# haoheliu/voicefixer

Hardware: AMD Instinct MI355X
Metric: seconds-of-44.1kHz-audio restored per wall-second (higher is better)
Workload: dtype f32

## Files before the change

### voicefixer_amd/csrc/vfx_common.h

```cpp
#pragma once
#include <hip/hip_runtime.h>
#include <stdint.h>
#include <atomic>
#include "../../include/vfx_hip.h"

extern __attribute__((visibility("hidden"))) std::atomic<uint64_t> g_vfx_launches;

#define VFX_LAUNCHED() (g_vfx_launches.fetch_add(1, std::memory_order_relaxed))

static inline int vfx_last_error() {
    hipError_t e = hipGetLastError();
    return e == hipSuccess ? VFX_OK : (int)e;
}

__attribute__((visibility("hidden"))) int vfx_zero_u32(void* p, size_t bytes, hipStream_t s);

#ifdef VFX_DEV
#include <stdlib.h>
#define VFX_DEV_ENV(name) getenv(name)
#else
#define VFX_DEV_ENV(name) (static_cast<const char*>(nullptr))
#endif

static inline bool vfx_aligned16(const void* p) { return (reinterpret_cast<uintptr_t>(p) & 15u) == 0; }

__device__ __forceinline__ float vfx_lrelu(float v, float slope) { return v > 0.f ? v : v * slope; }

__device__ __forceinline__ float vfx_post(float v, int act, float slope) {
    switch (act) {
        case VFX_POST_LRELU: return vfx_lrelu(v, slope);
        case VFX_POST_ELU: return v > 0.f ? v : expm1f(v);
        case VFX_POST_TANH: return tanhf(v);
        case VFX_POST_SIGMOID: return 1.f / (1.f + expf(-v));
        case VFX_POST_LRELU_SNAKE: { float u = vfx_lrelu(v, slope); return u + sinf(u); }
        default: return v;
    }
}
```

### voicefixer_amd/csrc/vfx_convwg.inc

```

static void convwg_fold_blocks(ConvArgs& a, dim3& grid, int gy) {
    static const bool off = VFX_DEV_ENV("VFX_WINO_MFOLD") && atoi(VFX_DEV_ENV("VFX_WINO_MFOLD")) == 0;
    a.nph_fold = 0;
    if (gy > 1 && a.xcd_chunk > 0 && !off) {
        a.nph_fold = gy;
        grid = dim3(grid.x * gy, 1, grid.z);
    }
}

#ifndef VFX_WG4_OCC
#define VFX_WG4_OCC 2
#endif
#ifndef VFX_WG4_ABL
#define VFX_WG4_ABL 0
#endif
#ifndef VFX_WG4_SPEC2_OCC
#define VFX_WG4_SPEC2_OCC 2
#endif
template <int WGM, int WGP, bool D1 = false, int XD = 2, bool PRE = true, int SPEC = 0>
__global__ __launch_bounds__(256, (SPEC == 2 && WGM == 4) ? VFX_WG4_SPEC2_OCC : VFX_WG4_OCC) void convwg4_kernel(const ConvArgs a) {
    static_assert(WGM * WGP == 4, "four waves");
    static_assert(SPEC == 0 || (SPEC == 1 && PRE) || (SPEC == 2 && D1 && !PRE), "specialised instances");
    constexpr bool ZSTART = SPEC != 0;
    static_assert(XD == 2 || XD == 3, "prefetch distance");
    constexpr int XSETS = XD - 1;
    constexpr int KC = 16, NSTEP = KC / 2;
    constexpr int BM = 32 * WGM, BQ = 32 * WGP;
    constexpr int CG = 256 / BQ;
    constexpr int NSLOT = KC / CG;
    constexpr int SPAN = NSTEP / NSLOT;
    constexpr int PLANE = KC * BQ;
    constexpr int BUF = 6 * PLANE;
    static_assert(CG % 2 == 0 && (SPAN == 2 || SPAN == 4), "staging map");
    extern __shared__ __attribute__((aligned(16))) float smem[];

    const int tid = threadIdx.x, lane = tid & 63;
    const int wave = __builtin_amdgcn_readfirstlane(tid >> 6);
    const int lo = lane & 31, hi = lane >> 5;
    const int wm = wave / WGP, wp = wave % WGP;
    int bx = blockIdx.x;
    int mblk = blockIdx.y;
    if (a.xcd_chunk > 0) {
        int k = bx >> 3;
        if (a.nph_fold > 1) {
            const int t = k / a.nph_fold;
            mblk = k - t * a.nph_fold;
            k = t;
        }
        bx = (bx & 7) * a.xcd_chunk + k;
        if (bx >= a.ntiles_l) return;
    }
    const int m0 = mblk * BM;
    const int b = blockIdx.z;
    const int d = D1 ? 1 : a.wg_d;
    const float inv_d = 1.0f / (float)d;
    const int Lrow = a.x_rows ? __builtin_amdgcn_readfirstlane(a.x_rows[b]) : a.Lin;
    const int Q0 = bx * BQ;
    {
        const int nblk = fast_div(Lrow + 4 * d - 1, 4 * d, 0.25f * inv_d);
        if (Q0 >= nblk * d) return;
    }
    if (a.stagger) {
        const int lin = blockIdx.x + gridDim.x * (blockIdx.y + gridDim.y * blockIdx.z);
        if (lin < a.stagger_wgs) {
            const int slot = __builtin_amdgcn_s_getreg((3 << 11) | 4) & 15;
            for (int i = 0; i < slot * a.stagger; ++i) __builtin_amdgcn_s_sleep(127);
        }
    }
    DBG_T(dbg_t0);
#if VFX_ABL & 8
    unsigned long long dbg_bar = 0;
#define WG4_SYNC() do { DBG_T(b0_); __syncthreads(); DBG_T(b1_); dbg_bar += b1_ - b0_; } while (0)
#else
#define WG4_SYNC() do { if (!(VFX_WG4_ABL & 16)) __syncthreads(); } while (0)
#endif
    const int xcs = (int)a.x_cs;
    auto quad_q = [&](int Q) {
        if constexpr (D1) return 4 * Q;
        const int blk = fast_div(Q, d, inv_d);
        return 4 * d * blk + (Q - blk * d);
    };
    const bool has_tail = D1 && (Lrow & 3) != 0 && (Lrow >> 2) >= Q0 && (Lrow >> 2) < Q0 + BQ;

    const int sq = tid % BQ, cg = tid / BQ;
    int xvoff[6];
    bool xin[4] = {true, true, true, true};
    {
        const int q = quad_q(Q0 + sq);
#pragma unroll
        for (int j = 0; j < 6; ++j) {
            const int p = q + (j - 1) * d;
            xvoff[j] = (p >= 0 && p < Lrow) ? (cg * xcs + p) * 4 : VFX_W_OOB;
        }
        if constexpr (D1) {
#pragma unroll
            for (int i = 0; i < 4; ++i) xin[i] = q + i < Lrow;
        }
    }
    const __amdgpu_buffer_rsrc_t xrsrc = __builtin_amdgcn_make_buffer_rsrc(
        const_cast<float*>(a.x) + (long long)b * a.x_bs, (short)0, 0x7fffffff, 0x00020000);
    const float slope = a.pre_act == VFX_PRE_LRELU ? a.pre_slope : 1.f;
    auto x_soff = [&](int v) { return v * KC * xcs * 4; };
    const int wcol = BQ == 32 ? sq : ((sq & ~63) | ((sq + 32 * (cg & 1)) & 63));
    float* const wbase = smem + cg * BQ + wcol;

    float xv[XSETS][NSLOT][6];
    auto x_load_part = [&](auto set_tag, int j, int part, int s0) {
        constexpr int SET = decltype(set_tag)::value;
        const int so = s0 + j * CG * xcs * 4;
        if constexpr (D1) {
            if (part == 0) {
                const u32x4 r = __builtin_amdgcn_raw_buffer_load_b128(xrsrc, xvoff[1], so, 0);
                xv[SET][j][1] = __uint_as_float(r.x); xv[SET][j][2] = __uint_as_float(r.y);
                xv[SET][j][3] = __uint_as_float(r.z); xv[SET][j][4] = __uint_as_float(r.w);
            } else if (part == 1) {
                xv[SET][j][0] = __uint_as_float(__builtin_amdgcn_raw_buffer_load_b32(xrsrc, xvoff[0], so, 0));
            } else if (part == 2) {
                xv[SET][j][5] = __uint_as_float(__builtin_amdgcn_raw_buffer_load_b32(xrsrc, xvoff[5], so, 0));
            }
        } else {
            xv[SET][j][part] = __uint_as_float(__builtin_amdgcn_raw_buffer_load_b32(xrsrc, xvoff[part], so, 0));
        }
    };
    auto x_load = [&](auto set_tag, int v) {
        const int s0 = x_soff(v);
#pragma unroll
        for (int j = 0; j < NSLOT; ++j)
#pragma unroll
            for (int t = 0; t < 6; ++t) x_load_part(set_tag, j, t, s0);
    };
    auto x_transform = [&](auto set_tag, int j, float (&V)[6]) {
        constexpr int SET = decltype(set_tag)::value;
        float e[6];
#pragma unroll
        for (int t = 0; t < 6; ++t) {
            e[t] = PRE ? fmaxf(xv[SET][j][t], xv[SET][j][t] * slope) : xv[SET][j][t];
            if constexpr (D1) {
                if (t >= 1 && t <= 4) e[t] = xin[t - 1] ? e[t] : 0.f;
            }
        }
        const float s1 = fmaf(-4.f, e[2], e[4]), s2 = fmaf(-4.f, e[1], e[3]);
        const float s3 = e[4] - e[2], s4 = e[3] - e[1];
        V[0] = fmaf(4.f, e[0], fmaf(-5.f, e[2], e[4]));
        V[1] = s1 + s2;
        V[2] = s1 - s2;
        V[3] = fmaf(2.f, s4, s3);
        V[4] = fmaf(-2.f, s4, s3);
        V[5] = fmaf(4.f, e[1], fmaf(-5.f, e[3], e[5]));
    };
    auto x_write = [&](auto set_tag, float* dst) {
#pragma unroll
        for (int j = 0; j < NSLOT; ++j) {
            float V[6];
            x_transform(set_tag, j, V);
#pragma unroll
            for (int k = 0; k < 6; ++k) dst[j * CG * BQ + k * PLANE] = V[k];
        }
    };

    const __amdgpu_buffer_rsrc_t wrsrc =
        __builtin_amdgcn_make_buffer_rsrc(const_cast<float*>(a.wd), (short)0, 0x7fffffff, 0x00020000);
    const int avoff = ((m0 + wm * 32 + lo) * 8 + 4 * hi) * 4;
    const int gstride = a.Cout * 32;
    const int pstride = (a.CinPad >> 3) * gstride;
    float4 aw[2][6];
    auto a_goff = [&](int vg) { return (VFX_WG4_ABL & 1) ? 0 : vg * gstride; };
    auto a_load_one = [&](auto set_tag, int k, int goff) {
        constexpr int SET = decltype(set_tag)::value;
        const u32x4 r = __builtin_amdgcn_raw_buffer_load_b128(wrsrc, avoff, k * pstride + goff, 0);
        aw[SET][k] = make_float4(__uint_as_float(r.x), __uint_as_float(r.y), __uint_as_float(r.z), __uint_as_float(r.w));
    };

    const int row0 = m0 + wm * 32;
    int rv[4];
    int rvq = VFX_W_OOB;
    {
        const int q = quad_q(Q0 + wp * 32 + lo);
#pragma unroll
        for (int i = 0; i < 4; ++i) rv[i] = q + i * d < Lrow ? (4 * hi * (int)a.r_cs + q + i * d) * 4 : VFX_W_OOB;
        if constexpr (D1) {
            const bool full = q + 3 < Lrow;
            rvq = (full && a.res) ? rv[0] : VFX_W_OOB;
#pragma unroll
            for (int i = 0; i < 4; ++i) rv[i] = full ? VFX_W_OOB : rv[i];
        }
    }
    f32x16 acc[6];
    u32x4 rq[(D1 && SPEC == 0) ? 16 : 1];
    const __amdgpu_buffer_rsrc_t rrsrc = __builtin_amdgcn_make_buffer_rsrc(
        const_cast<float*>(a.res ? a.res : a.x) + (long long)b * a.r_bs, (short)0, 0x7fffffff, 0x00020000);
    const __amdgpu_buffer_rsrc_t brsrc = __builtin_amdgcn_make_buffer_rsrc(
        const_cast<float*>(a.bias ? a.bias : a.x), (short)0, 0x7fffffff, 0x00020000);
    u32x4 bq[4];
    {
        const int bvoff = a.bias ? (row0 + 4 * hi) * 4 : VFX_W_OOB;
#pragma unroll
        for (int g = 0; g < 4; ++g) bq[g] = __builtin_amdgcn_raw_buffer_load_b128(brsrc, bvoff, g * 32, 0);
    }
    using X0 = std::integral_constant<int, 0>;
    using X1 = std::integral_constant<int, XSETS - 1>;
#if VFX_ABL & 8
    __builtin_amdgcn_sched_barrier(0);
#endif
    DBG_T(dbg_tr);
#if VFX_ABL & 8
    __builtin_amdgcn_sched_barrier(0);
#endif
    x_load(X0{}, 0);
#pragma unroll
    for (int k = 0; k < 6; ++k) a_load_one(std::integral_constant<int, 0>{}, k, a_goff(0));
#if VFX_ABL & 8
    __builtin_amdgcn_sched_barrier(0);
#endif
    DBG_T(dbg_ts);
#if VFX_ABL & 8
    __builtin_amdgcn_sched_barrier(0);
#endif
    if constexpr (SPEC == 0) {
        const int cs4 = (int)a.r_cs * 4;
        if constexpr (D1) {
#pragma unroll
            for (int r = 0; r < 16; ++r)
                rq[r] = __builtin_amdgcn_raw_buffer_load_b128(rrsrc, rvq, (row0 + (r & 3) + 8 * (r >> 2)) * cs4, 0);
        } else if (a.res) {
#pragma unroll
            for (int r = 0; r < 16; ++r) {
                const int soff = (row0 + (r & 3) + 8 * (r >> 2)) * cs4;
                acc[0][r] = __uint_as_float(__builtin_amdgcn_raw_buffer_load_b32(rrsrc, rv[0], soff, 0));
                acc[1][r] = __uint_as_float(__builtin_amdgcn_raw_buffer_load_b32(rrsrc, rv[1], soff, 0));
                acc[3][r] = __uint_as_float(__builtin_amdgcn_raw_buffer_load_b32(rrsrc, rv[2], soff, 0));
                acc[5][r] = __uint_as_float(__builtin_amdgcn_raw_buffer_load_b32(rrsrc, rv[3], soff, 0));
            }
        } else {
#pragma unroll
            for (int r = 0; r < 16; ++r) { acc[0][r] = 0.f; acc[1][r] = 0.f; acc[3][r] = 0.f; acc[5][r] = 0.f; }
        }
    }
    __builtin_amdgcn_sched_barrier(0);
    DBG_T(dbg_ta);
    auto acc_start = [&]() {
        if constexpr (ZSTART) return;
        if constexpr (D1 && SPEC == 0) {
#pragma unroll
            for (int r = 0; r < 16; ++r) {
                acc[0][r] = __uint_as_float(rq[r].x); acc[1][r] = __uint_as_float(rq[r].y);
                acc[3][r] = __uint_as_float(rq[r].z); acc[5][r] = __uint_as_float(rq[r].w);
            }
        }
        if (D1 && has_tail && a.res) {
            const int cs4 = (int)a.r_cs * 4;
#pragma unroll 1
            for (int r = 0; r < 16; ++r) {
                const int soff = (row0 + (r & 3) + 8 * (r >> 2)) * cs4;
                const float t0 = __uint_as_float(__builtin_amdgcn_raw_buffer_load_b32(rrsrc, rv[0], soff, 0));
                const float t1 = __uint_as_float(__builtin_amdgcn_raw_buffer_load_b32(rrsrc, rv[1], soff, 0));
                const float t2 = __uint_as_float(__builtin_amdgcn_raw_buffer_load_b32(rrsrc, rv[2], soff, 0));
                const float t3 = __uint_as_float(__builtin_amdgcn_raw_buffer_load_b32(rrsrc, rv[3], soff, 0));
                acc[0][r] += t0; acc[1][r] += t1; acc[3][r] += t2; acc[5][r] += t3;
            }
        }
        if (!a.res) {
#pragma unroll
            for (int g = 0; g < 4; ++g)
#pragma unroll
                for (int e = 0; e < 4; ++e) {
                    const int r = 4 * g + e;
                    acc[0][r] = 0.f;
                    acc[1][r] = __uint_as_float(e == 0 ? bq[g].x : (e == 1 ? bq[g].y : (e == 2 ? bq[g].z : bq[g].w)));
                    acc[2][r] = 0.f; acc[3][r] = 0.f; acc[4][r] = 0.f; acc[5][r] = 0.f;
                }
            return;
        }
#pragma unroll
        for (int g = 0; g < 4; ++g) {
#pragma unroll
            for (int e = 0; e < 4; ++e) {
                const int r = 4 * g + e;
                const float bb = __uint_as_float(e == 0 ? bq[g].x : (e == 1 ? bq[g].y : (e == 2 ? bq[g].z : bq[g].w)));
                const float t0 = acc[0][r] + bb, t1 = acc[1][r] + bb, t2 = acc[3][r] + bb, t3 = acc[5][r] + bb;
                const float m3 = 0.5f * (t2 - t1);
                const float m1 = 2.f * t1 - t2;
                acc[0][r] = t0 - m1 - m3;
                acc[1][r] = m1;
                acc[2][r] = 0.f;
                acc[3][r] = m3;
                acc[4][r] = 0.f;
                acc[5][r] = t3 - m1 - 8.f * m3;
            }
        }
    };

    const int bcol = BQ == 32 ? lo : ((wp * 32 + lo + 32 * hi) & 63);
    const int boffs = hi * BQ + bcol;

    f32x16 biasv;
    if constexpr (ZSTART) {
#pragma unroll
        for (int g = 0; g < 4; ++g) {
            biasv[4 * g + 0] = __uint_as_float(bq[g].x); biasv[4 * g + 1] = __uint_as_float(bq[g].y);
            biasv[4 * g + 2] = __uint_as_float(bq[g].z); biasv[4 * g + 3] = __uint_as_float(bq[g].w);
        }
    }
    auto mma_chunk = [&](auto set_tag, auto first_tag, const float* xs, float* wdst, int xchunk, int agrp0, int glast) {
        constexpr bool FIRST = decltype(first_tag)::value;
        const float* bp = xs + boffs;
        const int agrp1 = a_goff(min(agrp0 + 1, glast)), agrp2 = a_goff(min(agrp0 + 2, glast));
        float bf[6];
#pragma unroll
        for (int k = 0; k < 6; ++k) bf[k] = bp[k * PLANE];
        const int xs0 = x_soff(xchunk);
        float V[6];
#pragma unroll
        for (int u = 0; u < NSTEP; ++u) {
            const int el = u / SPAN, ph = u % SPAN;
#pragma unroll
            for (int k = 0; k < 6; ++k) {
                constexpr bool ST = !(VFX_WG4_ABL & 8), LD = !(VFX_WG4_ABL & 2);
                if constexpr (SPAN == 4) {
                    if (ST && ph == 0 && k == 0) x_transform(set_tag, el, V);
                    if (ST && ph == 0 && k < 3) wdst[el * CG * BQ + k * PLANE] = V[k];
                    if (ST && ph == 1 && k < 3) wdst[el * CG * BQ + (k + 3) * PLANE] = V[k + 3];
                    if (LD && ph == 2 && k < 3) x_load_part(set_tag, el, k, xs0);
                    if (LD && ph == 3 && k < 3) x_load_part(set_tag, el, k + 3, xs0);
                } else {
                    if (ST && ph == 0 && k == 0) x_transform(set_tag, el, V);
                    if (ST && ph == 0) wdst[el * CG * BQ + k * PLANE] = V[k];
                    if (LD && ph == 1) x_load_part(set_tag, el, k, xs0);
                }
                if (u == 0) a_load_one(std::integral_constant<int, 1>{}, k, agrp1);
                if (u == 4) a_load_one(std::integral_constant<int, 0>{}, k, agrp2);
                const float4 av4 = (u < 4) ? aw[0][k] : aw[1][k];
                const int kk = u & 3;
                const float av = kk == 0 ? av4.x : (kk == 1 ? av4.y : (kk == 2 ? av4.z : av4.w));
                if constexpr (FIRST) {
                    if (u == 0) {
                        const f32x16 zero16 = {0.f, 0.f, 0.f, 0.f, 0.f, 0.f, 0.f, 0.f, 0.f, 0.f, 0.f, 0.f, 0.f, 0.f, 0.f, 0.f};
                        acc[k] = __builtin_amdgcn_mfma_f32_32x32x2f32(av, bf[k], k == 1 ? biasv : zero16, 0, 0, 0);
                    } else {
                        acc[k] = __builtin_amdgcn_mfma_f32_32x32x2f32(av, bf[k], acc[k], 0, 0, 0);
                    }
                } else {
                    acc[k] = __builtin_amdgcn_mfma_f32_32x32x2f32(av, bf[k], acc[k], 0, 0, 0);
                }
                if (u < NSTEP - 1 && !(VFX_WG4_ABL & 4)) bf[k] = bp[k * PLANE + (u + 1) * 2 * BQ];
                __builtin_amdgcn_sched_barrier(0);
            }
        }
    };

    const int S = a.Cin / KC;
    const int glast = 2 * S - 1;
    x_write(X0{}, wbase);
    DBG_T(dbg_tb);
    x_load(X0{}, S > 1 ? 1 : 0);
    if constexpr (XSETS == 2) x_load(X1{}, min(2, S - 1));
    __builtin_amdgcn_sched_barrier(0);
    acc_start();
    DBG_T(dbg_tc);
    WG4_SYNC();
    DBG_T(dbg_t1);
    using NotFirst = std::false_type;
    int s_begin = 0;
    if constexpr (ZSTART) {
        mma_chunk(X0{}, std::true_type{}, smem, wbase + BUF, min(XD, S - 1), 0, glast);
        WG4_SYNC();
        mma_chunk(X1{}, NotFirst{}, smem + BUF, wbase, min(1 + XD, S - 1), 2, glast);
        WG4_SYNC();
        s_begin = 2;
    }
#pragma unroll 1
    for (int s = s_begin; s < S; s += 2) {
        mma_chunk(X0{}, NotFirst{}, smem, wbase + BUF, min(s + XD, S - 1), 2 * s, glast);
        WG4_SYNC();
        mma_chunk(X1{}, NotFirst{}, smem + BUF, wbase, min(s + 1 + XD, S - 1), 2 * s + 2, glast);
        WG4_SYNC();
    }
    DBG_T(dbg_t2);

    const __amdgpu_buffer_rsrc_t yrsrc = __builtin_amdgcn_make_buffer_rsrc(
        a.y + (long long)b * a.y_bs, (short)0, 0x7fffffff, 0x00020000);
    const int ycs4 = (int)a.y_cs * 4;
    const int post = a.post_act;
    const float ps = a.post_slope;
    int yv[4];
    int yvq = VFX_W_OOB;
    {
        const int q = quad_q(Q0 + wp * 32 + lo);
#pragma unroll
        for (int i = 0; i < 4; ++i) yv[i] = q + i * d < Lrow ? (4 * hi * (int)a.y_cs + q + i * d) * 4 : VFX_W_OOB;
        if constexpr (D1) {
            const bool full = q + 3 < Lrow;
            yvq = full ? yv[0] : VFX_W_OOB;
#pragma unroll
            for (int i = 0; i < 4; ++i) yv[i] = full ? VFX_W_OOB : yv[i];
        }
    }
    auto store4 = [&](const float (&v)[4], int soff) {
        if constexpr (D1) {
            u32x4 u;
            u.x = __float_as_uint(v[0]); u.y = __float_as_uint(v[1]); u.z = __float_as_uint(v[2]); u.w = __float_as_uint(v[3]);
            __builtin_amdgcn_raw_buffer_store_b128(u, yrsrc, yvq, soff, 0);
        }
        if (!D1 || has_tail) {
#pragma unroll
            for (int i = 0; i < 4; ++i) __builtin_amdgcn_raw_buffer_store_b32(__float_as_uint(v[i]), yrsrc, yv[i], soff, 0);
        }
    };
    auto outs = [&](int r, float (&y)[4]) {
        const float p12 = acc[1][r] + acc[2][r], m12 = acc[1][r] - acc[2][r];
        const float p34 = acc[3][r] + acc[4][r], m34 = acc[3][r] - acc[4][r];
        y[0] = (acc[0][r] + p12) + p34;
        y[1] = fmaf(2.f, m34, m12);
        y[2] = fmaf(4.f, p34, p12);
        y[3] = fmaf(8.f, m34, m12) + acc[5][r];
    };
    if constexpr (SPEC == 1) {
#pragma unroll
        for (int r = 0; r < 16; ++r) {
            const int soff = (row0 + (r & 3) + 8 * (r >> 2)) * ycs4;
            float y[4];
            outs(r, y);
#pragma unroll
            for (int i = 0; i < 4; ++i) y[i] = fmaxf(y[i], y[i] * ps);
            store4(y, soff);
        }
    } else if constexpr (SPEC == 2) {
        const int cs4 = (int)a.r_cs * 4;
        const int qe = quad_q(Q0 + wp * 32 + lo);
        const bool full = qe + 3 < Lrow;
        const int rvq2 = full ? (4 * hi * (int)a.r_cs + qe) * 4 : VFX_W_OOB;
        int tv[4];
#pragma unroll
        for (int i = 0; i < 4; ++i) tv[i] = (qe + i < Lrow && !full) ? (4 * hi * (int)a.r_cs + qe + i) * 4 : VFX_W_OOB;
        u32x4 rl[2][4];
        auto res_load = [&](int bt, u32x4 (&dst)[4]) {
#pragma unroll
            for (int e = 0; e < 4; ++e) dst[e] = __builtin_amdgcn_raw_buffer_load_b128(rrsrc, rvq2, (row0 + e + 8 * bt) * cs4, 0);
        };
        res_load(0, rl[0]);
        res_load(1, rl[1]);
        __builtin_amdgcn_sched_barrier(0);
#pragma unroll
        for (int bt = 0; bt < 4; ++bt) {
#pragma unroll
            for (int e = 0; e < 4; ++e) {
                const int r = 4 * bt + e;
                const int srow = row0 + e + 8 * bt;
                float y[4];
                outs(r, y);
                const u32x4 t = rl[bt & 1][e];
                y[0] += __uint_as_float(t.x); y[1] += __uint_as_float(t.y); y[2] += __uint_as_float(t.z); y[3] += __uint_as_float(t.w);
                if (has_tail) {
#pragma unroll
                    for (int i = 0; i < 4; ++i) y[i] += __uint_as_float(__builtin_amdgcn_raw_buffer_load_b32(rrsrc, tv[i], srow * cs4, 0));
                }
                store4(y, srow * ycs4);
            }
            if (bt + 2 < 4) res_load(bt + 2, rl[bt & 1]);
            __builtin_amdgcn_sched_barrier(0);
        }
    } else if (post == VFX_POST_NONE) {
#pragma unroll
        for (int r = 0; r < 16; ++r) {
            const int soff = (row0 + (r & 3) + 8 * (r >> 2)) * ycs4;
            float y[4];
            outs(r, y);
            store4(y, soff);
        }
    } else if (post == VFX_POST_LRELU) {
#pragma unroll
        for (int r = 0; r < 16; ++r) {
            const int soff = (row0 + (r & 3) + 8 * (r >> 2)) * ycs4;
            float y[4];
            outs(r, y);
#pragma unroll
            for (int i = 0; i < 4; ++i) y[i] = fmaxf(y[i], y[i] * ps);
            store4(y, soff);
        }
    } else {
#pragma unroll 1
        for (int r = 0; r < 16; ++r) {
            const int soff = (row0 + (r & 3) + 8 * (r >> 2)) * ycs4;
            float y[4];
            outs(r, y);
#pragma unroll
            for (int i = 0; i < 4; ++i) y[i] = vfx_post(y[i], post, ps);
            store4(y, soff);
        }
    }
#undef WG4_SYNC
#if VFX_ABL & 8
    DBG_T(dbg_t3);
    if (tid == 0 && g_trace_buf) {
        const unsigned long long lin = blockIdx.x + (unsigned long long)gridDim.x * (blockIdx.y + gridDim.y * blockIdx.z);
        if (lin < g_trace_cap) {
            unsigned long long* t = g_trace_buf + 6ull * lin;
            t[0] = (unsigned long long)(unsigned)__builtin_amdgcn_s_getreg((31 << 11) | 4) |
                   ((unsigned long long)(unsigned)__builtin_amdgcn_s_getreg((31 << 11) | 20) << 32);
            t[1] = lin + 1;
            t[2] = dbg_t0; t[3] = dbg_t1; t[4] = dbg_t2; t[5] = dbg_t3;
        }
    } else if (tid == 0) {
        atomicAdd(&g_dbg[8], dbg_t1 - dbg_t0);
        atomicAdd(&g_dbg[0], dbg_ta - dbg_t0);
        atomicAdd(&g_dbgx[0], dbg_tr - dbg_t0);
        atomicAdd(&g_dbgx[1], dbg_ta - dbg_ts);
        atomicAdd(&g_dbgx[2], dbg_ts - dbg_tr);
        atomicAdd(&g_dbg[1], dbg_tb - dbg_ta);
        atomicAdd(&g_dbg[2], dbg_tc - dbg_tb);
        atomicAdd(&g_dbg[9], dbg_t1 - dbg_tc - (dbg_bar ? 0 : 0));
        atomicAdd(&g_dbg[4], dbg_t2 - dbg_t1);
        atomicAdd(&g_dbg[5], dbg_t3 - dbg_t2);
        atomicAdd(&g_dbg[3], dbg_bar);
        atomicAdd(&g_dbg[6], 1ull);
        atomicAdd(&g_dbg[7], (unsigned long long)S);
    }
#endif
}

template <int WGM, int WGP, bool D1 = false, int XD = 2, bool PRE = true, int SPEC = 0>
static int launch_wg4_xd(const ConvArgs& a, dim3 grid, size_t lds, hipStream_t s) {
    static unsigned long long attr_set = 0;
    int attr_dev = 0;
    if (hipGetDevice(&attr_dev) != hipSuccess) attr_dev = 0;
    auto kern = convwg4_kernel<WGM, WGP, D1, XD, PRE, SPEC>;
    if (!((attr_set >> (attr_dev & 63)) & 1ull)) {
        hipError_t e = hipFuncSetAttribute(reinterpret_cast<const void*>(kern),
                                           hipFuncAttributeMaxDynamicSharedMemorySize, 160 * 1024);
        if (e != hipSuccess) return (int)e;
        attr_set |= 1ull << (attr_dev & 63);
    }
    hipLaunchKernelGGL(kern, grid, dim3(256), lds, s, a);
    VFX_LAUNCHED();
    return vfx_last_error();
}

template <int WGM, int WGP, bool D1 = false>
static int launch_wg4_one(const ConvArgs& a, dim3 grid, size_t lds, hipStream_t s) {
#ifdef VFX_DEV
    static const int xd = VFX_DEV_ENV("VFX_WG4_XD") ? atoi(VFX_DEV_ENV("VFX_WG4_XD")) : 2;
    if (xd == 3) return launch_wg4_xd<WGM, WGP, D1, 3, true>(a, grid, lds, s);
    static const int spec_mask = VFX_DEV_ENV("VFX_WG4_SPEC") ? atoi(VFX_DEV_ENV("VFX_WG4_SPEC")) : 3;
#else
    constexpr int spec_mask = 3;
#endif
    if ((spec_mask & 1) && !a.res && a.pre_act == VFX_PRE_LRELU && a.post_act == VFX_POST_LRELU && (!a.bias || vfx_aligned16(a.bias)))
        return launch_wg4_xd<WGM, WGP, D1, 2, true, 1>(a, grid, lds, s);
    if constexpr (D1) {
        if ((spec_mask & 2) && a.res && a.pre_act == VFX_PRE_NONE && a.post_act == VFX_POST_NONE && (!a.bias || vfx_aligned16(a.bias)))
            return launch_wg4_xd<WGM, WGP, true, 2, false, 2>(a, grid, lds, s);
    }
    return a.pre_act == VFX_PRE_NONE ? launch_wg4_xd<WGM, WGP, D1, 2, false>(a, grid, lds, s)
                                     : launch_wg4_xd<WGM, WGP, D1, 2, true>(a, grid, lds, s);
}

static int try_launch_convwg4p(ConvArgs a, int ntiles, int gy, bool wide, bool d1vec, hipStream_t stream);
static int try_launch_convwg4x(ConvArgs a, long long nquads, bool d1vec, hipStream_t stream);
#ifndef VFX_WG4X_DEFAULT
#define VFX_WG4X_DEFAULT 1
#endif

static int try_launch_convwg4(ConvArgs a, const vfx_tensor* x, int nphase, const PhaseSpec* phs, const float* wg4,
                              hipStream_t stream) {
    static const bool off = (VFX_DEV_ENV("VFX_WINO") && atoi(VFX_DEV_ENV("VFX_WINO")) == 0) ||
                            (VFX_DEV_ENV("VFX_WINO4") && atoi(VFX_DEV_ENV("VFX_WINO4")) == 0);
    if (off || !wg4 || !vfx_aligned16(wg4)) return VFX_ENOTSUP;
    if (nphase != 1 || phs[0].ntaps != 3 || phs[0].ooff != 0) return VFX_ENOTSUP;
    const int d = phs[0].taps[2].off;
    if (d < 1 || phs[0].taps[0].off != -d || phs[0].taps[1].off != 0) return VFX_ENOTSUP;
    for (int t = 0; t < 3; ++t)
        if (phs[0].taps[t].slab != t) return VFX_ENOTSUP;
    if (a.pad_mode != VFX_PAD_ZERO || a.in_mask || a.out_mask) return VFX_ENOTSUP;
    if (a.pre_act != VFX_PRE_NONE && a.pre_act != VFX_PRE_LRELU) return VFX_ENOTSUP;
    if (a.pre_act == VFX_PRE_LRELU && !(a.pre_slope >= 0.f && a.pre_slope <= 1.f)) return VFX_ENOTSUP;
    if (a.post_act == VFX_POST_LRELU && !(a.post_slope >= 0.f && a.post_slope <= 1.f)) return VFX_ENOTSUP;
    if (a.q_shift != 31 || a.o_rs != 0 || a.o_cs != 1 || a.y_ls != 1 || a.Lq != a.Lin || a.Lq > a.Lout) return VFX_ENOTSUP;
    if (a.res && a.r_ls != 1) return VFX_ENOTSUP;
    if (a.Cin % 32 != 0 || a.Cout % 64 != 0 || a.Cin != a.CinPad) return VFX_ENOTSUP;
    static const bool square = VFX_DEV_ENV("VFX_WINO4_SQUARE") && atoi(VFX_DEV_ENV("VFX_WINO4_SQUARE")) != 0;
    const bool wide = a.Cout % 128 == 0 && !square;
    {
        const long long lim = (1ll << 31) - (1ll << 20);
        if (((long long)a.Cin * a.x_cs + a.Lin) * 4 >= lim || ((long long)a.Cout * a.y_cs + a.Lout) * 4 >= lim ||
            (a.res && ((long long)a.Cout * a.r_cs + a.Lout) * 4 >= lim))
            return VFX_ENOTSUP;
        if (6ll * (a.CinPad >> 3) * a.Cout * 32 >= lim) return VFX_ENOTSUP;
    }
    const long long nquads = ((long long)a.Lin + 4 * d - 1) / (4 * d) * d;
    const int BQ = wide ? 32 : 64;
    const int ntiles = (int)((nquads + BQ - 1) / BQ);
    const int gy = a.Cout / (wide ? 128 : 64);
    if ((long long)ntiles * gy * a.B < 512) return VFX_ENOTSUP;
    a.wd = wg4;
    a.wg_d = d;
    a.x_guard = 0;
    a.tab = nullptr;
    a.stagger = 0; a.stagger_wgs = 0;
    if (VFX_DEV_ENV("VFX_WG4_STAGGER")) {
        a.stagger = atoi(VFX_DEV_ENV("VFX_WG4_STAGGER"));
        a.stagger_wgs = 256 * 3;
    }
    if (!a.res) { a.r_bs = a.x_bs; a.r_cs = a.x_cs; }
    size_t lds = 2ull * 6 * 16 * BQ * sizeof(float);
    if (VFX_DEV_ENV("VFX_WG4_LDS_PAD_KB"))
        lds += (size_t)atoi(VFX_DEV_ENV("VFX_WG4_LDS_PAD_KB")) * 1024;
    dim3 grid(convw_grid_x(a, ntiles), gy, a.B);
    convwg_fold_blocks(a, grid, gy);
    g_last_tile = (wide ? 128 : 64) * 100000 + 4 * BQ * 100 + 80;
    static const bool d1_off = VFX_DEV_ENV("VFX_WINO4_D1") && atoi(VFX_DEV_ENV("VFX_WINO4_D1")) == 0;
    const bool vec_ok = ((a.x_cs | a.x_bs | a.y_cs | a.y_bs) & 3) == 0 && vfx_aligned16(a.x) && vfx_aligned16(a.y) &&
                        (!a.res || (((a.r_cs | a.r_bs) & 3) == 0 && vfx_aligned16(a.res)));
    const bool d1vec = d == 1 && vec_ok && !d1_off;
    static const int wg4x = VFX_DEV_ENV("VFX_WG4X") ? atoi(VFX_DEV_ENV("VFX_WG4X")) : VFX_WG4X_DEFAULT;
    if (wide && wg4x && (wg4x != 2 || d1vec || a.Cout == 128)) {
        const int rc = try_launch_convwg4x(a, nquads, d1vec, stream);
        if (rc != VFX_ENOTSUP) {
            if (rc == VFX_OK) g_last_tile = 128 * 100000 + 256 * 100 + 82;
            return rc;
        }
    }
    {
        const int rc = try_launch_convwg4p(a, ntiles, gy, wide, d1vec, stream);
        if (rc != VFX_ENOTSUP) {
            if (rc == VFX_OK) g_last_tile = (wide ? 128 : 64) * 100000 + 4 * BQ * 100 + 81;
            return rc;
        }
    }
    if (d1vec)
        return wide ? launch_wg4_one<4, 1, true>(a, grid, lds, stream) : launch_wg4_one<2, 2, true>(a, grid, lds, stream);
    return wide ? launch_wg4_one<4, 1>(a, grid, lds, stream) : launch_wg4_one<2, 2>(a, grid, lds, stream);
}
```

### voicefixer_amd/csrc/vfx_convwg4x.inc

```
#ifndef VFX_WG4X_ABL
#define VFX_WG4X_ABL 0
#endif
template <bool D1, bool PRE, int SPEC>
__global__ __launch_bounds__(256, 1) void convwg4x_kernel(const ConvArgs a) {
    static_assert((SPEC == 1 && PRE) || (SPEC == 2 && D1 && !PRE), "specialised instances only");
    constexpr int KC = 8, NSTEP = KC / 2;
    constexpr int BM = 128, BQ = 64;
    constexpr int CG = 256 / BQ;
    constexpr int NSLOT = KC / CG;
    constexpr int SPAN = NSTEP / NSLOT;
    constexpr int PLANE = KC * BQ;
    constexpr int BUF = 6 * PLANE;
    constexpr int OBUF = 32 * 4 * BQ;
    constexpr int TPK = D1 ? 1 : 4;
    constexpr int NSL = NSTEP * TPK;
    constexpr int NUNIT = D1 ? 32 : 128;
    constexpr int NIT = NUNIT / NSL;
    static_assert(NIT * NSL == NUNIT && NIT == 8, "an iteration is valid or not as a whole");
    static_assert(SPAN == 2, "staging map");
    extern __shared__ __attribute__((aligned(16))) float smem[];

    const int tid = threadIdx.x, lane = tid & 63;
    const int wave = __builtin_amdgcn_readfirstlane(tid >> 6);
    const int lo = lane & 31, hi = lane >> 5;
    const int gy = a.nph_fold;
    const int per = gridDim.x >> 3;
    const int xcd = blockIdx.x & 7, jw = blockIdx.x >> 3;
    const int nend = min(a.B * a.ntiles_l * gy, (xcd + 1) * a.xcd_chunk);
    int n = xcd * a.xcd_chunk + jw;
    if (n >= nend) return;
    const int m0 = (jw % gy) * BM;
    const int d = D1 ? 1 : a.wg_d;
    const float inv_d = 1.0f / (float)d;
    const int xcs = (int)a.x_cs;
    const int S = a.Cin / KC;
    auto quad_q = [&](int Q) {
        if constexpr (D1) return 4 * Q;
        const int blk = fast_div(Q, d, inv_d);
        return 4 * d * blk + (Q - blk * d);
    };
    const int sq = lane, cg = wave;

    int t_b = 0, t_Q0 = 0, t_Lrow = 0, u_b = 0, u_Q0 = 0, u_Lrow = 0;
    bool t_valid = false, u_valid = false;
    auto tile_uniform = [&](int nn, int& b_, int& Q0_, int& Lrow_, bool& valid_) {
        valid_ = nn < nend;
        const int u = (valid_ ? nn : n) / gy;
        b_ = u / a.ntiles_l;
        Q0_ = (u - b_ * a.ntiles_l) * BQ;
        Lrow_ = a.x_rows ? __builtin_amdgcn_readfirstlane(a.x_rows[b_]) : a.Lin;
        const int nblk = fast_div(Lrow_ + 4 * d - 1, 4 * d, 0.25f * inv_d);
        valid_ = valid_ && Q0_ < nblk * d;
    };
    int xvoff[6];
    bool xin[4] = {true, true, true, true};
    bool xin_st[4] = {true, true, true, true};
    auto tile_thread = [&](int Q0_, int Lrow_, bool valid_) {
        const int q = quad_q(Q0_ + sq);
#pragma unroll
        for (int j = 0; j < 6; ++j) {
            const int p = q + (j - 1) * d;
            xvoff[j] = (valid_ && p >= 0 && p < Lrow_) ? (cg * xcs + p) * 4 : VFX_W_OOB;
        }
        if constexpr (D1) {
#pragma unroll
            for (int i = 0; i < 4; ++i) xin[i] = q + i < Lrow_;
        }
    };
    auto x_rsrc = [&](int b_) {
        return __builtin_amdgcn_make_buffer_rsrc(const_cast<float*>(a.x) + (long long)b_ * a.x_bs, (short)0, 0x7fffffff, 0x00020000);
    };
    const float slope = a.pre_slope;
    auto x_soff = [&](int v) { return v * KC * xcs * 4; };
    float* const wbase = smem + cg * BQ + 2 * (sq & 31) + (sq >> 5);
    float* const obuf = smem + 2 * BUF + wave * OBUF;

    float xv[2][NSLOT][6];
    auto x_load_part = [&](const int xset, const __amdgpu_buffer_rsrc_t& rs, int j, int part, int s0) {
        const int so = s0 + j * CG * xcs * 4;
        if constexpr (D1) {
            if (part == 0) {
                const u32x4 r = __builtin_amdgcn_raw_buffer_load_b128(rs, xvoff[1], so, 0);
                xv[xset][j][1] = __uint_as_float(r.x); xv[xset][j][2] = __uint_as_float(r.y);
                xv[xset][j][3] = __uint_as_float(r.z); xv[xset][j][4] = __uint_as_float(r.w);
            } else if (part == 1) {
                xv[xset][j][0] = __uint_as_float(__builtin_amdgcn_raw_buffer_load_b32(rs, xvoff[0], so, 0));
            } else if (part == 2) {
                xv[xset][j][5] = __uint_as_float(__builtin_amdgcn_raw_buffer_load_b32(rs, xvoff[5], so, 0));
            }
        } else {
            xv[xset][j][part] = __uint_as_float(__builtin_amdgcn_raw_buffer_load_b32(rs, xvoff[part], so, 0));
        }
    };
    auto x_load = [&](const int xset, const __amdgpu_buffer_rsrc_t& rs, int v) {
        const int s0 = x_soff(v);
#pragma unroll
        for (int j = 0; j < NSLOT; ++j)
#pragma unroll
            for (int p = 0; p < 6; ++p) x_load_part(xset, rs, j, p, s0);
    };
    auto x_transform = [&](const int xset, int j, float (&V)[6]) {
        float e[6];
#pragma unroll
        for (int p = 0; p < 6; ++p) {
            e[p] = PRE ? fmaxf(xv[xset][j][p], xv[xset][j][p] * slope) : xv[xset][j][p];
            if constexpr (D1) {
                if (p >= 1 && p <= 4) e[p] = xin_st[p - 1] ? e[p] : 0.f;
            }
        }
        const float s1 = fmaf(-4.f, e[2], e[4]), s2 = fmaf(-4.f, e[1], e[3]);
        const float s3 = e[4] - e[2], s4 = e[3] - e[1];
        V[0] = fmaf(4.f, e[0], fmaf(-5.f, e[2], e[4]));
        V[1] = s1 + s2;
        V[2] = s1 - s2;
        V[3] = fmaf(2.f, s4, s3);
        V[4] = fmaf(-2.f, s4, s3);
        V[5] = fmaf(4.f, e[1], fmaf(-5.f, e[3], e[5]));
    };

    const __amdgpu_buffer_rsrc_t wrsrc =
        __builtin_amdgcn_make_buffer_rsrc(const_cast<float*>(a.wd), (short)0, 0x7fffffff, 0x00020000);
    const int row0 = m0 + wave * 32;
    const int avoff = ((row0 + lo) * 8 + 4 * hi) * 4;
    const int gstride = a.Cout * 32;
    const int pstride = (a.CinPad >> 3) * gstride;
    float4 aw[2][6];
    auto a_goff = [&](int vg) { return (VFX_WG4X_ABL & 8) ? 0 : (vg >= S ? vg - S : vg) * gstride; };
    auto a_load_one = [&](auto set_tag, int k, int goff) {
        constexpr int SET = decltype(set_tag)::value;
        const u32x4 r = __builtin_amdgcn_raw_buffer_load_b128(wrsrc, avoff, k * pstride + goff, 0);
        aw[SET][k] = make_float4(__uint_as_float(r.x), __uint_as_float(r.y), __uint_as_float(r.z), __uint_as_float(r.w));
    };
    using A0 = std::integral_constant<int, 0>;
    using A1 = std::integral_constant<int, 1>;

    const float bias_a = (a.bias && hi == 0) ? a.bias[row0 + lo] : 0.f;
    f32x16 acc[6][2];
    const int boffs = hi * BQ + 2 * lo;
    const int cs4r = (int)a.r_cs * 4;
    const int ycs4 = (int)a.y_cs * 4;
    const float ps = a.post_slope;

    int tm = 0x1000000;
    int pyv[4] = {VFX_W_OOB, VFX_W_OOB, VFX_W_OOB, VFX_W_OOB};
    int pq4 = 0, p_Lrow4 = 0;
    float tl[NSL][D1 ? 4 : 1];
    u32x4 tres[SPEC == 2 ? NSL : 1];
    const float* p_ybase = a.y;
    const float* p_rbase = a.res ? a.res : a.x;
    struct TrickleIter {
        __amdgpu_buffer_rsrc_t yrs, rrs;
        int soff_u, soff_l;
        const float* yrow;
        const float* rrow;
        int nrec_u, nrec_l;
        const float* lds;
    };
    auto trickle_pending = [&]() { return tm <= NIT; };
    auto trickle_iter = [&]() {
        TrickleIter it;
        const bool ok_u = tm >= 1 && tm <= NIT, ok_l = tm < NIT;
        const int ml = ok_l ? tm : 0;
        it.yrs = __builtin_amdgcn_make_buffer_rsrc(const_cast<float*>(p_ybase), (short)0, ok_u ? 0x7fffffff : 0, 0x00020000);
        it.rrs = __builtin_amdgcn_make_buffer_rsrc(const_cast<float*>(p_rbase), (short)0, ok_l ? 0x7fffffff : 0, 0x00020000);
        it.soff_u = ok_u ? (row0 + (tm - 1) * 4) * ycs4 : 0;
        it.soff_l = (row0 + ml * 4) * cs4r;
        it.yrow = p_ybase + (long long)(row0 + (ok_u ? tm - 1 : 0) * 4) * a.y_cs;
        it.rrow = p_rbase + (long long)(row0 + ml * 4) * a.r_cs;
        it.nrec_u = ok_u ? p_Lrow4 : 0;
        it.nrec_l = ok_l ? p_Lrow4 : 0;
        it.lds = obuf + ml * (4 * 4 * BQ) + (D1 ? lane * 4 : lane);
        return it;
    };
    auto trickle_slot = [&](const TrickleIter& it, const int J) {
        if constexpr ((VFX_WG4X_ABL & 17) != 0) return;
        const int soff = it.soff_u + (D1 ? J : (J >> 2)) * ycs4;
        if constexpr (D1) {
            float y[4] = {tl[J][0], tl[J][1], tl[J][2], tl[J][3]};
            if constexpr (SPEC == 2) {
                y[0] += __uint_as_float(tres[J].x); y[1] += __uint_as_float(tres[J].y);
                y[2] += __uint_as_float(tres[J].z); y[3] += __uint_as_float(tres[J].w);
            } else {
#pragma unroll
                for (int i = 0; i < 4; ++i) y[i] = fmaxf(y[i], y[i] * ps);
            }
            u32x4 v;
            v.x = __float_as_uint(y[0]); v.y = __float_as_uint(y[1]); v.z = __float_as_uint(y[2]); v.w = __float_as_uint(y[3]);
            if constexpr (!(VFX_WG4X_ABL & 32)) {
                const __amdgpu_buffer_rsrc_t yr = __builtin_amdgcn_make_buffer_rsrc(const_cast<float*>(it.yrow + (long long)J * a.y_cs), (short)0, it.nrec_u, 0x00020000);
                __builtin_amdgcn_raw_buffer_store_b128(v, yr, pq4, 0, 0);
            } else if (y[0] + y[1] + y[2] + y[3] == 12345.678f) a.y[1] = y[0];
            const float4 nv = *reinterpret_cast<const float4*>(it.lds + J * (4 * BQ));
            tl[J][0] = nv.x; tl[J][1] = nv.y; tl[J][2] = nv.z; tl[J][3] = nv.w;
            if constexpr (SPEC == 2 && !(VFX_WG4X_ABL & 64)) {
                const __amdgpu_buffer_rsrc_t rr = __builtin_amdgcn_make_buffer_rsrc(const_cast<float*>(it.rrow + (long long)J * a.r_cs), (short)0, it.nrec_l, 0x00020000);
                tres[J] = __builtin_amdgcn_raw_buffer_load_b128(rr, pq4, 0, 0);
            }
        } else {
            float y = tl[J][0];
            y = fmaxf(y, y * ps);
            if constexpr (!(VFX_WG4X_ABL & 32)) __builtin_amdgcn_raw_buffer_store_b32(__float_as_uint(y), it.yrs, pyv[J & 3], soff, 0);
            else if (y == 12345.678f) a.y[1] = y;
            tl[J][0] = it.lds[J * BQ];
        }
    };
    auto trickle_drain = [&]() {
        while (trickle_pending()) {
            const TrickleIter it = trickle_iter();
#pragma unroll
            for (int j = 0; j < NSL; ++j) trickle_slot(it, j);
            ++tm;
        }
    };

    float2 bf[6];
    auto bf_first = [&](const float* xs) {
#pragma unroll
        for (int k = 0; k < 6; ++k) bf[k] = *reinterpret_cast<const float2*>(xs + boffs + k * PLANE);
    };
    auto mma_chunk = [&](auto first_tag, auto set_tag, auto trk_tag, const __amdgpu_buffer_rsrc_t& rsl, const float* xs, float* wdst, int xchunk, int agrp) {
        constexpr bool FIRST = decltype(first_tag)::value;
        constexpr bool TRK = decltype(trk_tag)::value;
        TrickleIter it;
        if constexpr (TRK) it = trickle_iter();
        constexpr int SET = decltype(set_tag)::value;
        const float* bp = xs + boffs;
        const float* bpn = (xs == smem ? smem + BUF : smem) + boffs;
        const int agn = a_goff(agrp + 1);
        const int xs0 = x_soff(xchunk);
        float V[6];
#pragma unroll
        for (int u = 0; u < NSTEP; ++u) {
            const int el = u / SPAN, ph = u % SPAN;
            if (u == NSTEP - 1 && !(VFX_WG4X_ABL & 4)) __syncthreads();
#pragma unroll
            for (int k = 0; k < 6; ++k) {
                constexpr bool STG = !(VFX_WG4X_ABL & 2);
                if (STG && ph == 0 && k == 0) x_transform(1 - SET, el, V);
                if (STG && ph == 0) wdst[el * CG * BQ + k * PLANE] = V[k];
                if (STG && ph == 1) x_load_part(1 - SET, rsl, el, k, xs0);
                if (u == 0) a_load_one(std::integral_constant<int, 1 - SET>{}, k, agn);
                const float4 av4 = aw[SET][k];
                const float av = u == 0 ? av4.x : (u == 1 ? av4.y : (u == 2 ? av4.z : av4.w));
                if constexpr (FIRST) {
                    if (u == 0) {
                        const f32x16 zero16 = {0.f, 0.f, 0.f, 0.f, 0.f, 0.f, 0.f, 0.f, 0.f, 0.f, 0.f, 0.f, 0.f, 0.f, 0.f, 0.f};
                        if (k == 1) {
                            acc[1][0] = __builtin_amdgcn_mfma_f32_32x32x2f32(bias_a, 1.0f, zero16, 0, 0, 0);
                            acc[1][1] = __builtin_amdgcn_mfma_f32_32x32x2f32(bias_a, 1.0f, zero16, 0, 0, 0);
                        }
                        acc[k][0] = __builtin_amdgcn_mfma_f32_32x32x2f32(av, bf[k].x, k == 1 ? acc[1][0] : zero16, 0, 0, 0);
                        __builtin_amdgcn_sched_barrier(0);
                        acc[k][1] = __builtin_amdgcn_mfma_f32_32x32x2f32(av, bf[k].y, k == 1 ? acc[1][1] : zero16, 0, 0, 0);
                    } else {
                        acc[k][0] = __builtin_amdgcn_mfma_f32_32x32x2f32(av, bf[k].x, acc[k][0], 0, 0, 0);
                        __builtin_amdgcn_sched_barrier(0);
                        acc[k][1] = __builtin_amdgcn_mfma_f32_32x32x2f32(av, bf[k].y, acc[k][1], 0, 0, 0);
                    }
                } else {
                    acc[k][0] = __builtin_amdgcn_mfma_f32_32x32x2f32(av, bf[k].x, acc[k][0], 0, 0, 0);
                    __builtin_amdgcn_sched_barrier(0);
                    acc[k][1] = __builtin_amdgcn_mfma_f32_32x32x2f32(av, bf[k].y, acc[k][1], 0, 0, 0);
                }
                if (u < NSTEP - 1) bf[k] = *reinterpret_cast<const float2*>(bp + k * PLANE + (u + 1) * 2 * BQ);
                else bf[k] = *reinterpret_cast<const float2*>(bpn + k * PLANE);
                __builtin_amdgcn_sched_barrier(0);
                if constexpr (TRK && TPK == 1) {
                    if (k == 2) trickle_slot(it, u);
                } else if constexpr (TRK) {
                    if (k != 0 && k != 3) trickle_slot(it, u * TPK + (k < 3 ? k - 1 : k - 2));
                }
                __builtin_amdgcn_sched_barrier(0);
            }
        }
        ++tm;
    };
    using Yes = std::true_type;
    using No = std::false_type;

    tile_uniform(n, t_b, t_Q0, t_Lrow, t_valid);
    bool restart = true;
#pragma unroll 1
    for (; n < nend; n += per) {
        tile_uniform(n + per, u_b, u_Q0, u_Lrow, u_valid);
        if (t_valid) {
            __amdgpu_buffer_rsrc_t xrs = x_rsrc(t_b);
            if (restart) {
                tile_thread(t_Q0, t_Lrow, true);
                if constexpr (D1) {
#pragma unroll
                    for (int i = 0; i < 4; ++i) xin_st[i] = xin[i];
                }
                x_load(0, xrs, 0);
#pragma unroll
                for (int k = 0; k < 6; ++k) a_load_one(A0{}, k, 0);
                __builtin_amdgcn_sched_barrier(0);
#pragma unroll
                for (int j = 0; j < NSLOT; ++j) {
                    float V[6];
                    x_transform(0, j, V);
#pragma unroll
                    for (int k = 0; k < 6; ++k) wbase[j * CG * BQ + k * PLANE] = V[k];
                }
                x_load(1, xrs, 1);
                x_load(0, xrs, 2);
                __builtin_amdgcn_sched_barrier(0);
                __syncthreads();
                bf_first(smem);
            }
            mma_chunk(Yes{}, A0{}, Yes{}, xrs, smem, wbase + BUF, 3, 0);
            mma_chunk(No{}, A1{}, Yes{}, xrs, smem + BUF, wbase, 4, 1);
            auto chunk_pair = [&](int s, auto trk_tag) {
                const bool last = s == S - 2;
                mma_chunk(No{}, A0{}, trk_tag, xrs, smem, wbase + BUF, last ? 1 : s + 3, s);
                if (s == S - 4) {
                    tile_thread(u_Q0, u_Lrow, u_valid);
                    xrs = x_rsrc(u_b);
                }
                if (last) {
                    if constexpr (D1) {
#pragma unroll
                        for (int i = 0; i < 4; ++i) xin_st[i] = xin[i];
                    }
                }
                mma_chunk(No{}, A1{}, trk_tag, xrs, smem + BUF, wbase, s >= S - 4 ? s + 4 - S : s + 4, s + 1);
            };
            const int SA = min(S, NIT + 2);
#pragma unroll 1
            for (int s = 2; s < SA; s += 2) chunk_pair(s, Yes{});
#pragma unroll 1
            for (int s = SA; s < S; s += 2) chunk_pair(s, No{});

            trickle_drain();
            if constexpr ((VFX_WG4X_ABL & 1) == 0) {
#pragma unroll
                for (int qb = 0; qb < 2; ++qb) {
#pragma unroll
                    for (int r = 0; r < 16; ++r) {
                        const float p12 = acc[1][qb][r] + acc[2][qb][r], m12 = acc[1][qb][r] - acc[2][qb][r];
                        const float p34 = acc[3][qb][r] + acc[4][qb][r], m34 = acc[3][qb][r] - acc[4][qb][r];
                        const float y0 = (acc[0][qb][r] + p12) + p34;
                        const float y1 = fmaf(2.f, m34, m12);
                        const float y2 = fmaf(4.f, p34, p12);
                        const float y3 = fmaf(8.f, m34, m12) + acc[5][qb][r];
                        const int rr = (r & 3) + 8 * (r >> 2);
                        if constexpr (D1) {
                            *reinterpret_cast<float4*>(obuf + ((rr + 4 * hi) * BQ + qb * 32 + lo) * 4) = make_float4(y0, y1, y2, y3);
                        } else {
                            float* o = obuf + (rr + 4 * hi) * 4 * BQ + qb * 32 + lo;
                            o[0 * BQ] = y0; o[1 * BQ] = y1; o[2 * BQ] = y2; o[3 * BQ] = y3;
                        }
                    }
                }
                p_ybase = a.y + (long long)t_b * a.y_bs;
                p_rbase = (a.res ? a.res : a.x) + (long long)t_b * a.r_bs;
                const int ql = quad_q(t_Q0 + lane);
                if constexpr (D1) {
                    pq4 = ql * 4;
                    p_Lrow4 = t_Lrow * 4;
                } else {
#pragma unroll
                    for (int i = 0; i < 4; ++i) pyv[i] = ql + i * d < t_Lrow ? (ql + i * d) * 4 : VFX_W_OOB;
                }
                tm = 0;
            } else {
                float sink = 0.f;
#pragma unroll
                for (int k = 0; k < 6; ++k) sink += acc[k][0][0] + acc[k][1][15];
                if (sink == 12345.678f) a.y[0] = sink;
            }
            restart = !u_valid;
        } else {
            restart = true;
        }
        t_b = u_b; t_Q0 = u_Q0; t_Lrow = u_Lrow; t_valid = u_valid;
    }
    trickle_drain();
}

template <bool D1, bool PRE, int SPEC>
static int launch_wg4x(const ConvArgs& a, int nwg, size_t lds, hipStream_t s) {
    static unsigned long long attr_set = 0;
    int attr_dev = 0;
    if (hipGetDevice(&attr_dev) != hipSuccess) attr_dev = 0;
    auto kern = convwg4x_kernel<D1, PRE, SPEC>;
    if (!((attr_set >> (attr_dev & 63)) & 1ull)) {
        hipError_t e = hipFuncSetAttribute(reinterpret_cast<const void*>(kern),
                                           hipFuncAttributeMaxDynamicSharedMemorySize, 160 * 1024);
        if (e != hipSuccess) return (int)e;
        attr_set |= 1ull << (attr_dev & 63);
    }
    hipLaunchKernelGGL(kern, dim3(nwg), dim3(256), lds, s, a);
    VFX_LAUNCHED();
    return vfx_last_error();
}

static int try_launch_convwg4x(ConvArgs a, long long nquads, bool d1vec, hipStream_t stream) {
    const int S = a.Cin / 8;
    if (S < 8 || (S & 1)) return VFX_ENOTSUP;
    if (a.Cout % 128 != 0) return VFX_ENOTSUP;
    if (a.bias && !vfx_aligned16(a.bias)) return VFX_ENOTSUP;
    const bool first = !a.res && a.pre_act == VFX_PRE_LRELU && a.post_act == VFX_POST_LRELU;
    const bool second = d1vec && a.res && a.pre_act == VFX_PRE_NONE && a.post_act == VFX_POST_NONE;
    if (!first && !second) return VFX_ENOTSUP;
    const int gy = a.Cout / 128;
    const int ntiles = (int)((nquads + 63) / 64);
    const long long N = (long long)a.B * ntiles * gy;
    if (N >= (1ll << 30)) return VFX_ENOTSUP;
    int nwg = vfx_cu_count();
    nwg -= nwg % (8 * gy);
    if (nwg < 8 * gy || N < 4ll * nwg) return VFX_ENOTSUP;
    long long chunk = (N + 7) / 8;
    chunk = (chunk + gy - 1) / gy * gy;
    a.ntiles_l = ntiles;
    a.nph_fold = gy;
    a.xcd_chunk = (int)chunk;
    const size_t lds = (2ull * 6 * 8 * 64 + 4ull * 32 * 256) * sizeof(float);
    if (first) return d1vec ? launch_wg4x<true, true, 1>(a, nwg, lds, stream) : launch_wg4x<false, true, 1>(a, nwg, lds, stream);
    return launch_wg4x<true, false, 2>(a, nwg, lds, stream);
}
```

Baseline: 1613.

## Fuse LReLU and snake post-activation into Winograd conv kernels with fast sine

```diff
diff --git a/voicefixer_amd/csrc/vfx_common.h b/voicefixer_amd/csrc/vfx_common.h
--- a/voicefixer_amd/csrc/vfx_common.h
+++ b/voicefixer_amd/csrc/vfx_common.h
@@ -26,13 +26,61 @@
 
 __device__ __forceinline__ float vfx_lrelu(float v, float slope) { return v > 0.f ? v : v * slope; }
 
+#define VFX_SNAKE_SIN_MAX 8192.0f
+
+__device__ __forceinline__ float vfx_snake_sin_fast(float x) {
+    const float ax = fabsf(x);
+    float kf = fmaf(ax, 0.636619772367581343f, 12582912.0f);
+    const unsigned q = __float_as_uint(kf);
+    kf -= 12582912.0f;
+    float r = fmaf(kf, -1.57079637050628662109375f, ax);
+    r = fmaf(kf, 4.37113882867379288655e-8f, r);
+    r = fmaf(kf, 1.71512451000588187280e-15f, r);
+    const float z = r * r;
+    const float sp = fmaf(fmaf(-1.9515295891e-4f, z, 8.3321608736e-3f), z, -1.6666654611e-1f);
+    const float s = fmaf(r * z, sp, r);
+    const float cp = fmaf(fmaf(2.443315711809948e-5f, z, -1.388731625493765e-3f), z, 4.166664568298827e-2f);
+    const float c = fmaf(z * z, cp, fmaf(-0.5f, z, 1.0f));
+    const float v = (q & 1u) ? c : s;
+    const unsigned sb = ((q << 30) ^ __float_as_uint(x)) & 0x80000000u;
+    return __uint_as_float(__float_as_uint(v) ^ sb);
+}
+
+__device__ __forceinline__ float vfx_snake_fast(float u, bool& wild) {
+    wild = wild || !(fabsf(u) <= VFX_SNAKE_SIN_MAX);
+    return u + vfx_snake_sin_fast(u);
+}
+
+template <int N>
+__device__ __forceinline__ void vfx_snake(float (&u)[N]) {
+    float y[N];
+    bool wild = false;
+#pragma unroll
+    for (int i = 0; i < N; ++i) y[i] = vfx_snake_fast(u[i], wild);
+    if (__builtin_expect(__any(wild), 0)) {
+#pragma unroll 1
+        for (int i = 0; i < N; ++i) {
+            float t = u[0];
+#pragma unroll
+            for (int j = 1; j < N; ++j) t = i == j ? u[j] : t;
+            if (!(fabsf(t) <= VFX_SNAKE_SIN_MAX)) {
+                const float v = t + sinf(t);
+#pragma unroll
+                for (int j = 0; j < N; ++j) y[j] = i == j ? v : y[j];
+            }
+        }
+    }
+#pragma unroll
+    for (int i = 0; i < N; ++i) u[i] = y[i];
+}
+
 __device__ __forceinline__ float vfx_post(float v, int act, float slope) {
     switch (act) {
         case VFX_POST_LRELU: return vfx_lrelu(v, slope);
         case VFX_POST_ELU: return v > 0.f ? v : expm1f(v);
         case VFX_POST_TANH: return tanhf(v);
         case VFX_POST_SIGMOID: return 1.f / (1.f + expf(-v));
-        case VFX_POST_LRELU_SNAKE: { float u = vfx_lrelu(v, slope); return u + sinf(u); }
+        case VFX_POST_LRELU_SNAKE: { float u[1] = {vfx_lrelu(v, slope)}; vfx_snake<1>(u); return u[0]; }
         default: return v;
     }
 }
diff --git a/voicefixer_amd/csrc/vfx_convwg.inc b/voicefixer_amd/csrc/vfx_convwg.inc
--- a/voicefixer_amd/csrc/vfx_convwg.inc
+++ b/voicefixer_amd/csrc/vfx_convwg.inc
@@ -477,6 +477,17 @@
             for (int i = 0; i < 4; ++i) y[i] = fmaxf(y[i], y[i] * ps);
             store4(y, soff);
         }
+    } else if (post == VFX_POST_LRELU_SNAKE) {
+#pragma unroll
+        for (int r = 0; r < 16; ++r) {
+            const int soff = (row0 + (r & 3) + 8 * (r >> 2)) * ycs4;
+            float y[4];
+            outs(r, y);
+#pragma unroll
+            for (int i = 0; i < 4; ++i) y[i] = fmaxf(y[i], y[i] * ps);
+            vfx_snake<4>(y);
+            store4(y, soff);
+        }
     } else {
 #pragma unroll 1
         for (int r = 0; r < 16; ++r) {
@@ -573,7 +584,7 @@
     if (a.pad_mode != VFX_PAD_ZERO || a.in_mask || a.out_mask) return VFX_ENOTSUP;
     if (a.pre_act != VFX_PRE_NONE && a.pre_act != VFX_PRE_LRELU) return VFX_ENOTSUP;
     if (a.pre_act == VFX_PRE_LRELU && !(a.pre_slope >= 0.f && a.pre_slope <= 1.f)) return VFX_ENOTSUP;
-    if (a.post_act == VFX_POST_LRELU && !(a.post_slope >= 0.f && a.post_slope <= 1.f)) return VFX_ENOTSUP;
+    if ((a.post_act == VFX_POST_LRELU || a.post_act == VFX_POST_LRELU_SNAKE) && !(a.post_slope >= 0.f && a.post_slope <= 1.f)) return VFX_ENOTSUP;
     if (a.q_shift != 31 || a.o_rs != 0 || a.o_cs != 1 || a.y_ls != 1 || a.Lq != a.Lin || a.Lq > a.Lout) return VFX_ENOTSUP;
     if (a.res && a.r_ls != 1) return VFX_ENOTSUP;
     if (a.Cin % 32 != 0 || a.Cout % 64 != 0 || a.Cin != a.CinPad) return VFX_ENOTSUP;
diff --git a/voicefixer_amd/csrc/vfx_convwg4x.inc b/voicefixer_amd/csrc/vfx_convwg4x.inc
--- a/voicefixer_amd/csrc/vfx_convwg4x.inc
+++ b/voicefixer_amd/csrc/vfx_convwg4x.inc
@@ -1,9 +1,10 @@
 #ifndef VFX_WG4X_ABL
 #define VFX_WG4X_ABL 0
 #endif
-template <bool D1, bool PRE, int SPEC>
+template <bool D1, bool PRE, int SPEC, int POST = VFX_POST_NONE>
 __global__ __launch_bounds__(256, 1) void convwg4x_kernel(const ConvArgs a) {
     static_assert((SPEC == 1 && PRE) || (SPEC == 2 && D1 && !PRE), "specialised instances only");
+    static_assert(POST == VFX_POST_NONE || (SPEC == 2 && (POST == VFX_POST_LRELU || POST == VFX_POST_LRELU_SNAKE)), "post-activation of the second convolution");
     constexpr int KC = 8, NSTEP = KC / 2;
     constexpr int BM = 128, BQ = 64;
     constexpr int CG = 256 / BQ;
@@ -180,6 +181,11 @@
             if constexpr (SPEC == 2) {
                 y[0] += __uint_as_float(tres[J].x); y[1] += __uint_as_float(tres[J].y);
                 y[2] += __uint_as_float(tres[J].z); y[3] += __uint_as_float(tres[J].w);
+                if constexpr (POST != VFX_POST_NONE) {
+#pragma unroll
+                    for (int i = 0; i < 4; ++i) y[i] = fmaxf(y[i], y[i] * ps);
+                }
+                if constexpr (POST == VFX_POST_LRELU_SNAKE) vfx_snake<4>(y);
             } else {
 #pragma unroll
                 for (int i = 0; i < 4; ++i) y[i] = fmaxf(y[i], y[i] * ps);
@@ -378,12 +384,12 @@
     trickle_drain();
 }
 
-template <bool D1, bool PRE, int SPEC>
+template <bool D1, bool PRE, int SPEC, int POST = VFX_POST_NONE>
 static int launch_wg4x(const ConvArgs& a, int nwg, size_t lds, hipStream_t s) {
     static unsigned long long attr_set = 0;
     int attr_dev = 0;
     if (hipGetDevice(&attr_dev) != hipSuccess) attr_dev = 0;
-    auto kern = convwg4x_kernel<D1, PRE, SPEC>;
+    auto kern = convwg4x_kernel<D1, PRE, SPEC, POST>;
     if (!((attr_set >> (attr_dev & 63)) & 1ull)) {
         hipError_t e = hipFuncSetAttribute(reinterpret_cast<const void*>(kern),
                                            hipFuncAttributeMaxDynamicSharedMemorySize, 160 * 1024);
@@ -401,7 +407,9 @@
     if (a.Cout % 128 != 0) return VFX_ENOTSUP;
     if (a.bias && !vfx_aligned16(a.bias)) return VFX_ENOTSUP;
     const bool first = !a.res && a.pre_act == VFX_PRE_LRELU && a.post_act == VFX_POST_LRELU;
-    const bool second = d1vec && a.res && a.pre_act == VFX_PRE_NONE && a.post_act == VFX_POST_NONE;
+    const bool post_ok = a.post_act == VFX_POST_NONE || a.post_act == VFX_POST_LRELU ||
+                         (a.post_act == VFX_POST_LRELU_SNAKE && a.Cin >= 512);
+    const bool second = d1vec && a.res && a.pre_act == VFX_PRE_NONE && post_ok;
     if (!first && !second) return VFX_ENOTSUP;
     const int gy = a.Cout / 128;
     const int ntiles = (int)((nquads + 63) / 64);
@@ -417,5 +425,7 @@
     a.xcd_chunk = (int)chunk;
     const size_t lds = (2ull * 6 * 8 * 64 + 4ull * 32 * 256) * sizeof(float);
     if (first) return d1vec ? launch_wg4x<true, true, 1>(a, nwg, lds, stream) : launch_wg4x<false, true, 1>(a, nwg, lds, stream);
+    if (a.post_act == VFX_POST_LRELU_SNAKE) return launch_wg4x<true, false, 2, VFX_POST_LRELU_SNAKE>(a, nwg, lds, stream);
+    if (a.post_act == VFX_POST_LRELU) return launch_wg4x<true, false, 2, VFX_POST_LRELU>(a, nwg, lds, stream);
     return launch_wg4x<true, false, 2>(a, nwg, lds, stream);
 }
```

Result: no change. 1621 (median of 6 runs) (+0.5%).
